# Bill9125/T2MS

Measured on AMD Instinct MI355X. Metric: generated series/sec (B=256, L=96, 1000-step DDPM), higher is better.
Workload: dtype f32; 1 GPU; configs[1]: DiT denoiser, 1000-step ddpm with CFG (2 forwards/step), B=256/GPU, L=96, cfg_scale=9.0, LA-VAE decode; Philox noise on device; hipGraph=on; sampler lanes=2 (part-batch chains on own streams, include/t2s.h t2s_sampler_set_lanes); global_batch=256, diffusion_steps=1000, parallelism=batch-shard x1, sampler_lanes=2

## Files before the change

### include/t2s.h

```cpp
#ifndef T2S_H
#define T2S_H

#include <stdint.h>

#ifdef __cplusplus
extern "C" {
#endif

#define T2S_OK 0
#define T2S_E_INVALID (-1)
#define T2S_E_HIP (-2)
#define T2S_E_STATE (-3)

#define T2S_D_MODEL 128
#define T2S_N_TOK 480
#define T2S_N_HEADS 4
#define T2S_HEAD_DIM 32
#define T2S_N_BLOCKS 4
#define T2S_LAT_C 64
#define T2S_LAT_W 30
#define T2S_LAT_ELEMS (T2S_LAT_C * T2S_LAT_W)

const char* t2s_last_error(void);
const char* t2s_version(void);

typedef struct t2s_dit t2s_dit;

typedef struct t2s_dit_block_weights {
    const float* qkv_w;
    const float* qkv_b;
    const float* proj_w;
    const float* proj_b;
    const float* fc1_w;
    const float* fc1_b;
    const float* fc2_w;
    const float* fc2_b;
    const float* ada_w;
    const float* ada_b;
} t2s_dit_block_weights;

typedef struct t2s_dit_weights {
    const float* conv_w;
    const float* conv_b;
    const float* patch_w;
    const float* patch_b;
    const float* pos_embed;
    const float* ln_w;
    const float* ln_b;
    const float* out_w;
    const float* out_b;
    const float* time_freqs;
    t2s_dit_block_weights blk[T2S_N_BLOCKS];
} t2s_dit_weights;

int t2s_dit_create(const t2s_dit_weights* w, int max_seqs, t2s_dit** out);
#define T2S_DIT_N_TENSORS (10 + 10 * T2S_N_BLOCKS)
int t2s_dit_weights_check(const t2s_dit_weights* w, const uint64_t* n_floats, int n_entries);
int t2s_dit_update_weights(t2s_dit* h, const t2s_dit_weights* w, void* stream);
void t2s_dit_destroy(t2s_dit* h);
int t2s_dit_max_seqs(const t2s_dit* h);
#define T2S_MATH_F32 0
#define T2S_MATH_BF16X3 1
#define T2S_MATH_BF16 2
int t2s_dit_set_math(t2s_dit* h, int math);

int t2s_time_embedding(const t2s_dit* h, const float* t, float* out, int B, void* stream);
int t2s_time_embedding_freqs(const float* freqs, const float* t, float* out, int B, void* stream);

int t2s_dit_forward(t2s_dit* h, const float* x, const float* temb, int temb_rows,
                    const float* text, float* out, int B, void* stream);

int t2s_dit_forward_cfg(t2s_dit* h, const float* x, const float* temb, const float* text,
                        float* out_uncond, float* out_cond, int B, void* stream);
int t2s_dit_forward_cfg_rows(t2s_dit* h, const float* x, const float* temb, int temb_rows, const float* text,
                             float* out_uncond, float* out_cond, int B, void* stream);

int t2s_dit_timing_begin(t2s_dit* h);
int t2s_dit_timing_end(t2s_dit* h, double* out6);
int t2s_dit_timing_end_ex(t2s_dit* h, double* out, int n_classes);

int t2s_dit_read_stream(const t2s_dit* h, float* out, int S, void* stream);

int t2s_attn_fwd(const float* q, const float* k, const float* v, float* o, int BH, void* stream);
int t2s_attn_fwd_packed(const float* q, const float* k, const float* vT, float* o, int n_seq,
                        void* stream);

int t2s_attn_fwd_x3(const float* q, const float* k, const float* v, float* o, int BH, void* stream);

int t2s_attn_fwd_bf16p(const float* q, const float* k, const float* v, float* o, int BH, void* stream);

typedef struct t2s_dit_block_grads {
    float *qkv_w, *qkv_b, *proj_w, *proj_b, *fc1_w, *fc1_b, *fc2_w, *fc2_b, *ada_w, *ada_b;
} t2s_dit_block_grads;
typedef struct t2s_dit_grads {
    float *conv_w, *conv_b, *patch_w, *patch_b, *ln_w, *ln_b, *out_w, *out_b;
    t2s_dit_block_grads blk[T2S_N_BLOCKS];
} t2s_dit_grads;

#define T2S_TRAIN_F32 0
#define T2S_TRAIN_BF16 1
int t2s_dit_set_train_dtype(t2s_dit* h, int dtype);
int t2s_dit_train_forward(t2s_dit* h, const t2s_dit_weights* w, const float* x, const float* temb,
                          int temb_rows, const float* text, float* out, int B, void* stream);
int t2s_attn_fwd_bf16(const float* q, const float* k, const float* v, float* o_rows, float* lse,
                      int n_seq, void* stream);
int t2s_dit_train_backward(t2s_dit* h, const float* dout, const t2s_dit_grads* g, int B, void* stream);
int t2s_dit_train_input_grad(t2s_dit* h, float* dinput, int B, void* stream);
int t2s_adamw_step(float* param, const float* grad, float* exp_avg, float* exp_avg_sq, uint64_t n,
                   float lr, float beta1, float beta2, float eps, float weight_decay, int step,
                   void* stream);
typedef struct t2s_adamw_tensor {
    float* param;
    const float* grad;
    float* exp_avg;
    float* exp_avg_sq;
    uint64_t n;
} t2s_adamw_tensor;
int t2s_adamw_step_multi(const t2s_adamw_tensor* table_dev, int n_tensors, uint64_t total_chunks, float lr,
                         float beta1, float beta2, float eps, float weight_decay, int step, void* stream);
int t2s_mse_backward(const float* a, const float* b, const float* grad_out, float* da, float* db,
                     uint64_t n, void* stream);

int t2s_ddpm_step(float* x, const float* eps_u, const float* eps_c, const float* noise,
                  const float* coef, int t_index, float cfg, uint64_t seed, uint32_t stream_id,
                  uint32_t row0, int B, void* stream);
int t2s_ddpm_p_sample(const float* xt, const float* eps_hat, const int32_t* t, const float* noise,
                      const float* coef, float* out, int B, int n_steps, void* stream);
int t2s_ddpm_p_sample_n(const float* xt, const float* eps_hat, const int32_t* t, const float* noise,
                        const float* coef, float* out, int B, int row_elems, int n_steps, void* stream);
int t2s_ddpm_q_sample_n(const float* x0, const float* eps, const int32_t* t, const float* sqrt_ab,
                        const float* sqrt_1mab, float* out, int B, int row_elems, int n_steps, void* stream);
#define T2S_MSE_SCRATCH_FLOATS 1024
int t2s_mse_ws(const float* a, const float* b, float* out, uint64_t n, float* scratch, void* stream);
int t2s_mse(const float* a, const float* b, float* out, uint64_t n, void* stream);
int t2s_rf_step(float* x, const float* v_u, const float* v_c, float cfg, float dt, int B,
                void* stream);
int t2s_ddpm_q_sample(const float* x0, const float* eps, const int32_t* t, const float* sqrt_ab,
                      const float* sqrt_1mab, float* out, int B, int n_steps, void* stream);
int t2s_rf_create_flow(const float* x1, const float* x0, const float* t, float* out, int B,
                       void* stream);
int t2s_philox_normal(float* out, uint64_t seed, uint32_t stream_id, uint32_t row0, int n_rows,
                      int row_elems, void* stream);
int t2s_philox_normal_rows(float* out, const uint64_t* seeds, const uint32_t* key_rows, uint32_t stream_id,
                           int n_rows, int row_elems, void* stream);
int t2s_philox_uniform(float* out, uint64_t seed, uint32_t stream_id, uint32_t row0, int n_rows,
                       int row_elems, void* stream);

typedef struct t2s_vae t2s_vae;

typedef struct t2s_vae_stack_weights {
    const float* conv3_w[4];
    const float* conv1_w[4];
} t2s_vae_stack_weights;

typedef struct t2s_vae_weights {
    int hidden;
    int res_hidden;
    int n_res_layers;
    int emb;
    const float* dec_conv1_w;
    const float* dec_conv1_b;
    t2s_vae_stack_weights dec_stack;
    const float* dec_ct1_w;
    const float* dec_ct1_b;
    const float* dec_ct2_w;
    const float* dec_ct2_b;
    const float* enc_conv1_w;
    const float* enc_conv1_b;
// ... 124 lines not shown
```

### t2ms_amd/_lib.py

```python
from __future__ import annotations

import ctypes as C
import os
from typing import Optional

import torch

_HERE = os.path.dirname(os.path.abspath(__file__))
LIB_PATH = os.environ.get("T2S_LIB", os.path.join(_HERE, "libt2s_hip.so"))

N_BLOCKS = 4
LAT_C, LAT_W, LAT = 64, 30, 1920
D_MODEL, N_TOK = 128, 480
TRAIN_F32, TRAIN_BF16 = 0, 1
MATH_F32, MATH_BF16X3, MATH_BF16 = 0, 1, 2
MATH_CODES = {"f32": MATH_F32, "bf16x3": MATH_BF16X3, "bf16": MATH_BF16}
DIT_N_TENSORS = 10 + 10 * N_BLOCKS
MSE_SCRATCH_FLOATS = 1024

c_float_p = C.c_void_p


class DitBlockWeights(C.Structure):
    _fields_ = [(n, C.c_void_p) for n in
# ... 38 lines not shown

TS2VEC_MAX_BLOCKS = 16


class Ts2vecWeights(C.Structure):
    _fields_ = [("input_dims", C.c_int), ("hidden", C.c_int), ("output_dims", C.c_int), ("depth", C.c_int),
                ("fc_w", C.c_void_p), ("fc_b", C.c_void_p),
                ("conv1_w", C.c_void_p * TS2VEC_MAX_BLOCKS), ("conv1_b", C.c_void_p * TS2VEC_MAX_BLOCKS),
                ("conv2_w", C.c_void_p * TS2VEC_MAX_BLOCKS), ("conv2_b", C.c_void_p * TS2VEC_MAX_BLOCKS),
                ("proj_w", C.c_void_p), ("proj_b", C.c_void_p)]


MLP_LAYERS, MLP_PACKED_FLOATS = 8, 397888
MLP_LAYER_FIELDS = (("value_w", "cross_attn.value.weight"), ("value_b", "cross_attn.value.bias"),
                    ("proj_w", "cross_attn.proj.weight"), ("proj_b", "cross_attn.proj.bias"),
                    ("norm2_w", "norm2.weight"), ("norm2_b", "norm2.bias"),
                    ("mlp0_w", "mlp.0.weight"), ("mlp0_b", "mlp.0.bias"), ("mlp2_w", "mlp.2.weight"), ("mlp2_b", "mlp.2.bias"),
                    ("pos0_w", "mlp2.0.weight"), ("pos0_b", "mlp2.0.bias"), ("pos2_w", "mlp2.2.weight"), ("pos2_b", "mlp2.2.bias"))


class MlpLayerWeights(C.Structure):
    _fields_ = [(f, C.c_void_p) for f, _ in MLP_LAYER_FIELDS]


class MlpWeights(C.Structure):
    _fields_ = [("layer", MlpLayerWeights * MLP_LAYERS)]


MLP_GRAD_PART_FLOATS = 391744


class MlpGrads(C.Structure):
    _fields_ = [("layer", MlpLayerWeights * MLP_LAYERS)]


class SampleConfig(C.Structure):
    _fields_ = [("mode", C.c_int), ("steps", C.c_int), ("cfg_scale", C.c_float), ("batch", C.c_int),
                ("length", C.c_int), ("use_graph", C.c_int), ("seed", C.c_uint64), ("row0", C.c_uint32),
                ("ddpm_coef", C.c_void_p), ("t_values", C.c_void_p)]


MODE_DDPM, MODE_RF = 0, 1

_VP, _I, _F, _U64, _U32 = C.c_void_p, C.c_int, C.c_float, C.c_uint64, C.c_uint32
SYMBOLS = {
    "t2s_last_error": (C.c_char_p, []),
    "t2s_version": (C.c_char_p, []),
    "t2s_dit_create": (_I, [C.POINTER(DitWeights), _I, C.POINTER(_VP)]),
    "t2s_dit_update_weights": (_I, [_VP, C.POINTER(DitWeights), _VP]),
    "t2s_dit_destroy": (None, [_VP]),
    "t2s_dit_max_seqs": (_I, [_VP]),
    "t2s_time_embedding": (_I, [_VP, _VP, _VP, _I, _VP]),
    "t2s_time_embedding_freqs": (_I, [_VP, _VP, _VP, _I, _VP]),
    "t2s_dit_weights_check": (_I, [C.POINTER(DitWeights), C.POINTER(C.c_uint64), _I]),
    "t2s_dit_forward": (_I, [_VP, _VP, _VP, _I, _VP, _VP, _I, _VP]),
    "t2s_dit_forward_cfg": (_I, [_VP, _VP, _VP, _VP, _VP, _VP, _I, _VP]),
    "t2s_dit_forward_cfg_rows": (_I, [_VP, _VP, _VP, _I, _VP, _VP, _VP, _I, _VP]),
    "t2s_dit_read_stream": (_I, [_VP, _VP, _I, _VP]),
    "t2s_dit_timing_begin": (_I, [_VP]),
    "t2s_dit_timing_end": (_I, [_VP, C.POINTER(C.c_double)]),
    "t2s_dit_timing_end_ex": (_I, [_VP, C.POINTER(C.c_double), _I]),
    "t2s_dit_set_train_dtype": (_I, [_VP, _I]),
    "t2s_dit_set_math": (_I, [_VP, _I]),
    "t2s_eval_mse_wape": (_I, [_VP, _VP, _VP, _VP, _I, _I, _VP]),
    "t2s_eval_mrr": (_I, [_VP, _VP, _VP, _VP, _VP, _I, _I, _I, _F, _VP]),
    "t2s_eval_ed": (_I, [_VP, _VP, _VP, _VP, _I, _I, _I, _VP]),
    "t2s_eval_crps": (_I, [_VP, _VP, _VP, _VP, _I, _I, _I, _I, _VP]),
    "t2s_eval_dtw": (_I, [_VP, _VP, _VP, _VP, _I, _I, _I, _VP]),
    "t2s_ts2vec_encode": (_I, [C.POINTER(Ts2vecWeights), _VP, _VP, _VP, _I, _I, _VP]),
    "t2s_mlp_pack": (_I, [C.POINTER(MlpWeights), _VP, _VP]),
    "t2s_mlp_forward": (_I, [_VP, _VP, _VP, _VP, _VP, _VP, _I, _VP]),
    "t2s_mlp_backward": (_I, [C.POINTER(MlpWeights), _VP, _VP, _VP, _VP, _VP, _VP, _VP, C.POINTER(MlpGrads), _VP, _U64, _I, _VP]),
    "t2s_attn_fwd_x3": (_I, [_VP, _VP, _VP, _VP, _I, _VP]),
    "t2s_attn_fwd_bf16p": (_I, [_VP, _VP, _VP, _VP, _I, _VP]),
    "t2s_attn_fwd_bf16": (_I, [_VP, _VP, _VP, _VP, _VP, _I, _VP]),
    "t2s_dit_train_forward": (_I, [_VP, C.POINTER(DitWeights), _VP, _VP, _I, _VP, _VP, _I, _VP]),
    "t2s_dit_train_backward": (_I, [_VP, _VP, C.POINTER(DitGrads), _I, _VP]),
    "t2s_dit_train_input_grad": (_I, [_VP, _VP, _I, _VP]),
    "t2s_adamw_step": (_I, [_VP, _VP, _VP, _VP, _U64, _F, _F, _F, _F, _F, _I, _VP]),
    "t2s_adamw_step_multi": (_I, [_VP, _I, _U64, _F, _F, _F, _F, _F, _I, _VP]),
    "t2s_mse_backward": (_I, [_VP, _VP, _VP, _VP, _VP, _U64, _VP]),
    "t2s_attn_fwd": (_I, [_VP, _VP, _VP, _VP, _I, _VP]),
    "t2s_attn_fwd_packed": (_I, [_VP, _VP, _VP, _VP, _I, _VP]),
    "t2s_ddpm_step": (_I, [_VP, _VP, _VP, _VP, _VP, _I, _F, _U64, _U32, _U32, _I, _VP]),
    "t2s_ddpm_p_sample": (_I, [_VP, _VP, _VP, _VP, _VP, _VP, _I, _I, _VP]),
    "t2s_ddpm_p_sample_n": (_I, [_VP, _VP, _VP, _VP, _VP, _VP, _I, _I, _I, _VP]),
    "t2s_ddpm_q_sample_n": (_I, [_VP, _VP, _VP, _VP, _VP, _VP, _I, _I, _I, _VP]),
    "t2s_vae_decode_w": (_I, [_VP, _VP, _VP, _VP, _I, _I, _I, _VP]),
    "t2s_mse": (_I, [_VP, _VP, _VP, _U64, _VP]),
    "t2s_mse_ws": (_I, [_VP, _VP, _VP, _U64, _VP, _VP]),
    "t2s_rf_step": (_I, [_VP, _VP, _VP, _F, _F, _I, _VP]),
    "t2s_ddpm_q_sample": (_I, [_VP, _VP, _VP, _VP, _VP, _VP, _I, _I, _VP]),
    "t2s_rf_create_flow": (_I, [_VP, _VP, _VP, _VP, _I, _VP]),
    "t2s_philox_normal": (_I, [_VP, _U64, _U32, _U32, _I, _I, _VP]),
    "t2s_philox_uniform": (_I, [_VP, _U64, _U32, _U32, _I, _I, _VP]),
    "t2s_vae_create": (_I, [C.POINTER(VaeWeights), C.POINTER(_VP)]),
    "t2s_vae_destroy": (None, [_VP]),
    "t2s_vae_update_weights": (_I, [_VP, C.POINTER(VaeWeights), _VP]),
    "t2s_vae_encode_backward": (_I, [_VP, _VP, _VP, _VP, C.POINTER(VaeEncGrads), _I, _I, _VP]),
    "t2s_vae_decode": (_I, [_VP, _VP, _VP, _VP, _I, _I, _VP]),
    "t2s_vae_encode": (_I, [_VP, _VP, _VP, _VP, _I, _I, _VP]),
    "t2s_sampler_create": (_I, [_VP, _VP, C.POINTER(SampleConfig), C.POINTER(_VP)]),
    "t2s_sampler_destroy": (None, [_VP]),
    "t2s_sampler_run": (_I, [_VP, _VP, _VP, _VP, _VP, _VP, _VP]),
    "t2s_sampler_set_lanes": (_I, [_VP, _I]),
    "t2s_sampler_set_loop_graph": (_I, [_VP, _I]),
    "t2s_sampler_set_row0": (_I, [_VP, _U32]),
    "t2s_sampler_set_rows": (_I, [_VP, _VP, _VP, _VP, _I]),
    "t2s_philox_normal_rows": (_I, [_VP, _VP, _VP, _U32, _I, _I, _VP]),
    "t2s_sampler_graph_lanes": (_I, [_VP]),
    "t2s_sampler_lane_pool": (_I, []),
}

_lib: Optional[C.CDLL] = None


class T2SError(RuntimeError):
    pass


def lib() -> C.CDLL:
    global _lib
    if _lib is None:
        if not os.path.exists(LIB_PATH):
            raise T2SError(
                f"{LIB_PATH} is missing: build it with `python -c 'import __graft_entry__ as g; g.build()'` "
                f"or `make -C t2ms_amd/csrc` (hipcc --offload-arch=gfx950).  There is no CPU fallback.")
        handle = C.CDLL(LIB_PATH)
        for name, (res, args) in SYMBOLS.items():
            fn = getattr(handle, name)
            fn.restype, fn.argtypes = res, args
        _lib = handle
    return _lib


def check(rc: int, what: str = "") -> None:
    if rc != 0:
        msg = lib().t2s_last_error().decode("utf-8", "replace")
        raise T2SError(f"{what or 't2s call'} failed (rc={rc}): {msg}")


def dev_ptr(t: Optional[torch.Tensor], name: str = "tensor", dtype=torch.float32) -> Optional[int]:
    if t is None:
        return None
    if not t.is_cuda:
        raise T2SError(f"{name} must live on a GPU (got device {t.device}); the HIP path has no CPU fallback")
    if t.dtype != dtype:
        raise T2SError(f"{name} must be {dtype} (got {t.dtype})")
    if not t.is_contiguous():
        raise T2SError(f"{name} must be contiguous")
    return t.data_ptr()


def as_f32(t: torch.Tensor) -> torch.Tensor:
    if t.dtype != torch.float32:
        t = t.float()
    return t.contiguous()


_DEVICE_LOCKS = {}


def device_lock(device) -> "threading.RLock":
    import threading
    return _DEVICE_LOCKS.setdefault(str(torch.device(device)), threading.RLock())

# ... 9 lines not shown
```

### t2ms_amd/csrc/t2s_attn.hip

```cpp
#include <stdlib.h>

#include "t2s_common.h"

namespace t2s {

struct SoftmaxState {
    float m_run;
    float l_lane;
};

__device__ __forceinline__ float pair_max(float v) {
    const auto r = __builtin_amdgcn_permlane32_swap(__float_as_uint(v), __float_as_uint(v), false, false);
    return fmaxf(__uint_as_float(r[0]), __uint_as_float(r[1]));
}
__device__ __forceinline__ float pair_sum(float v) {
    const auto r = __builtin_amdgcn_permlane32_swap(__float_as_uint(v), __float_as_uint(v), false, false);
    return __uint_as_float(r[0]) + __uint_as_float(r[1]);
}

__device__ __forceinline__ void softmax_block(f32x16& st, f32x16& ot, SoftmaxState& s) {
    float mloc = st[0];
#pragma unroll
    for (int r = 1; r < 16; ++r) mloc = fmaxf(mloc, st[r]);
    mloc = pair_max(mloc);
    const float m_new = fmaxf(s.m_run, mloc);
    const float alpha = __builtin_amdgcn_exp2f(s.m_run - m_new);
    s.m_run = m_new;
    float psum = 0.f;
#pragma unroll
    for (int r = 0; r < 16; ++r) {
        st[r] = __builtin_amdgcn_exp2f(st[r] - m_new);
        psum += st[r];
    }
    s.l_lane = s.l_lane * alpha + psum;
#pragma unroll
    for (int r = 0; r < 16; ++r) ot[r] *= alpha;
}

constexpr float QSCALE = 0.17677669529663687f * 1.4426950408889634f;

constexpr int ATT_SLOTS = 4;
constexpr int ATT_SLOT_F4 = 512;
constexpr int ATT_LDS_BYTES = ATT_SLOTS * ATT_SLOT_F4 * 16;
constexpr int NKB = NTOK / 32;

constexpr float SM_BIG = 1.152921504606847e18f;


struct TileState {
    f32x16 negm;
    float m_ref;
    float l_lane;
};

__device__ __forceinline__ float exp_sum(f32x16& st) {
#pragma unroll
    for (int r = 0; r < 16; ++r) st[r] = __builtin_amdgcn_exp2f(st[r]);
    return ((st[0] + st[1]) + (st[2] + st[3])) + ((st[4] + st[5]) + (st[6] + st[7])) +
           (((st[8] + st[9]) + (st[10] + st[11])) + ((st[12] + st[13]) + (st[14] + st[15])));
}

__device__ __forceinline__ float rereference(const f32x4 (&kf)[4], const f32x4 (&q)[4], f32x16& st,
                                             f32x16& ot, TileState& t) {
#pragma unroll
    for (int r = 0; r < 16; ++r) st[r] = 0.f;
#pragma unroll
    for (int g = 0; g < 4; ++g)
#pragma unroll
        for (int e = 0; e < 4; ++e) st = mfma32(kf[g][e], q[g][e], st);
    float mloc = st[0];
#pragma unroll
    for (int r = 1; r < 16; ++r) mloc = fmaxf(mloc, st[r]);
    mloc = pair_max(mloc);
    const float m_new = fmaxf(t.m_ref, mloc);
    const float alpha = __builtin_amdgcn_exp2f(t.m_ref - m_new);
    t.m_ref = m_new;
    t.l_lane *= alpha;
#pragma unroll
    for (int r = 0; r < 16; ++r) {
        ot[r] *= alpha;
        t.negm[r] = -m_new;
        st[r] -= m_new;
    }
    return exp_sum(st);
}
// ... 218 lines not shown
                        sta = mfma32(kf[g][e], qa[g][e], sta);
                        if (NT == 2) stb = mfma32(kf[g][e], qb[g][e], stb);
                    }
                psa = exp_sum(sta);
                if (NT == 2) psb = exp_sum(stb);
                const bool stale = !(psa < SM_BIG) || !(psb < SM_BIG);
                redo = __builtin_amdgcn_ballot_w64(stale) != 0;
            }
            if (redo) {
                psa = rereference(kf, qa, sta, oa, ta);
                if (NT == 2) psb = rereference(kf, qb, stb, ob, tb);
            }
            ta.l_lane += psa;
            tb.l_lane += psb;
#pragma unroll
            for (int g = 0; g < 4; ++g)
#pragma unroll
                for (int e = 0; e < 4; ++e) oa = mfma32(vf[g][e], sta[4 * g + e], oa);
            if (jb == NKB - 4 && bh + stride < BH) {
                const f32x4* qg = qall + (size_t)(bh + stride) * NKB * 256;
#pragma unroll
                for (int g = 0; g < 4; ++g) {
                    qna[g] = qg[(t0 * 4 + g) * 64 + lane];
                    if (NT == 2) qnb[g] = qg[((t0 + 1) * 4 + g) * 64 + lane];
                }
            }
            ATT_PERSIST_WAIT();
            __builtin_amdgcn_s_barrier();
            issue_block(bh, jb + 4, gb + 4);
            {
                const f32x4* nslot = ring + ((gb + 1) & (ATT_SLOTS - 1)) * ATT_SLOT_F4 + lane;
#pragma unroll
                for (int g = 0; g < 4; ++g) kf[g] = nslot[g * 64];
            }
            if (NT == 2) {
#pragma unroll
                for (int g = 0; g < 4; ++g)
#pragma unroll
                    for (int e = 0; e < 4; ++e) ob = mfma32(vf[g][e], stb[4 * g + e], ob);
            }
        }
        const int seq = bh / NH, head = bh % NH;
        {
            const float inv = 1.0f / pair_sum(ta.l_lane);
#pragma unroll
            for (int g = 0; g < 4; ++g) {
                const f32x4 w = {oa[4 * g] * inv, oa[4 * g + 1] * inv, oa[4 * g + 2] * inv, oa[4 * g + 3] * inv};
                og[(((size_t)seq * NKB + t0) * 16 + head * 4 + g) * 64 + lane] = w;
            }
        }
        if (NT == 2) {
            const float inv = 1.0f / pair_sum(tb.l_lane);
#pragma unroll
            for (int g = 0; g < 4; ++g) {
                const f32x4 w = {ob[4 * g] * inv, ob[4 * g + 1] * inv, ob[4 * g + 2] * inv, ob[4 * g + 3] * inv};
                og[(((size_t)seq * NKB + t0 + 1) * 16 + head * 4 + g) * 64 + lane] = w;
            }
        }
#pragma unroll
        for (int g = 0; g < 4; ++g) {
            qa[g] = qna[g] * QSCALE;
            if (NT == 2) qb[g] = qnb[g] * QSCALE;
        }
    }
    asm volatile("s_waitcnt vmcnt(0)" ::: "memory");
}

__global__ __launch_bounds__(PERSIST_THREADS, 2) void attn_fwd_persistent_kernel(
    const float* __restrict__ q, const float* __restrict__ k, const float* __restrict__ vT,
    float* __restrict__ o, int BH) {
    extern __shared__ __attribute__((aligned(16))) f32x4 ring[];
    const int lane = threadIdx.x & 63;
    const int wave = __builtin_amdgcn_readfirstlane(threadIdx.x >> 6);
    const f32x4* qg = reinterpret_cast<const f32x4*>(q);
    const f32x4* kg = reinterpret_cast<const f32x4*>(k);
    const f32x4* vg = reinterpret_cast<const f32x4*>(vT);
    f32x4* og = reinterpret_cast<f32x4*>(o);
    if (wave < 7)
        attn_persistent_body<2>(ring, qg, kg, vg, og, BH, lane, wave);
    else
        attn_persistent_body<1>(ring, qg, kg, vg, og, BH, lane, wave);
}

int launch_attn_packed(const float* q, const float* k, const float* vT, float* o, int BH, hipStream_t st) {
    static int n_cu = 0;
    if (n_cu == 0) {
        int dev = 0;
        hipDeviceProp_t prop;
        if (hipGetDevice(&dev) == hipSuccess && hipGetDeviceProperties(&prop, dev) == hipSuccess)
            n_cu = prop.multiProcessorCount;
        else
            n_cu = 256;
    }
    static const int persist_min = getenv("T2S_ATTN_PERSIST_MIN") ? atoi(getenv("T2S_ATTN_PERSIST_MIN")) : 0;
    if (BH >= (persist_min > 0 ? persist_min : 3 * n_cu)) {
        attn_fwd_persistent_kernel<<<BH < n_cu ? BH : n_cu, PERSIST_THREADS, ATT_LDS_BYTES, st>>>(q, k, vT, o, BH);
    } else {
        static const int parts_env = getenv("T2S_ATTN_PARTS") ? atoi(getenv("T2S_ATTN_PARTS")) : 0;
        const int parts = parts_env == 2 || parts_env == 4 ? parts_env : (((BH + 7) / 8) * 16 < n_cu ? 4 : 2);
        if (parts == 4)
            attn_fwd_packed_kernel<4><<<((BH + 7) / 8) * 32, 256, ATT_LDS_BYTES, st>>>(q, k, vT, o, BH);
        else
            attn_fwd_packed_kernel<2><<<((BH + 7) / 8) * 16, 256, ATT_LDS_BYTES, st>>>(q, k, vT, o, BH);
    }
    T2S_LAUNCH_CHECK();
    return T2S_OK;
}

constexpr int KSTR = 36;
constexpr int PLAIN_LDS_BYTES = (NTOK * KSTR + NTOK * DH) * 4;

__global__ __launch_bounds__(512) void attn_fwd_plain_kernel(const float* __restrict__ q,
                                                             const float* __restrict__ k,
                                                             const float* __restrict__ v,
                                                             float* __restrict__ o) {
    extern __shared__ __attribute__((aligned(16))) float smem[];
    float* Ks = smem;
    float* Vs = smem + NTOK * KSTR;
    const int bh = blockIdx.x;
    const int tid = threadIdx.x;
    const int lane = tid & 63, wave = tid >> 6, half = lane >> 5, i = lane & 31;
    const float* kg = k + (size_t)bh * NTOK * DH;
    const float* vg = v + (size_t)bh * NTOK * DH;
    const float* qg = q + (size_t)bh * NTOK * DH;
    for (int idx = tid; idx < NTOK * DH / 4; idx += 512) {
        const f32x4 kv = reinterpret_cast<const f32x4*>(kg)[idx];
        const f32x4 vv = reinterpret_cast<const f32x4*>(vg)[idx];
        const int row = idx >> 3, col = (idx & 7) * 4;
        *reinterpret_cast<f32x4*>(Ks + row * KSTR + col) = kv;
        *reinterpret_cast<f32x4*>(Vs + row * DH + col) = vv;
    }
    __syncthreads();
    for (int qt = wave; qt < NKB; qt += 8) {
        f32x4 qf[4];
#pragma unroll
        for (int g = 0; g < 4; ++g)
            qf[g] = *reinterpret_cast<const f32x4*>(qg + (size_t)(qt * 32 + i) * DH + 8 * g + 4 * half) * QSCALE;
        f32x16 ot;
#pragma unroll
        for (int r = 0; r < 16; ++r) ot[r] = 0.f;
        SoftmaxState s{-INFINITY, 0.f};
        for (int jb = 0; jb < NKB; ++jb) {
            f32x16 st;
#pragma unroll
            for (int r = 0; r < 16; ++r) st[r] = 0.f;
            const float* krow = Ks + (jb * 32 + i) * KSTR + 4 * half;
#pragma unroll
            for (int g = 0; g < 4; ++g) {
                const f32x4 kf = *reinterpret_cast<const f32x4*>(krow + 8 * g);
#pragma unroll
                for (int e = 0; e < 4; ++e) st = mfma32(kf[e], qf[g][e], st);
            }
            softmax_block(st, ot, s);
            const float* vrow = Vs + (jb * 32 + 4 * half) * DH + i;
#pragma unroll
            for (int r = 0; r < 16; ++r) {
                const int klo = (r & 3) + 8 * (r >> 2);
                ot = mfma32(vrow[klo * DH], st[r], ot);
            }
        }
        const float inv = 1.0f / pair_sum(s.l_lane);
#pragma unroll
        for (int g = 0; g < 4; ++g) {
            const f32x4 w = {ot[4 * g] * inv, ot[4 * g + 1] * inv, ot[4 * g + 2] * inv, ot[4 * g + 3] * inv};
            *reinterpret_cast<f32x4*>(o + ((size_t)bh * NTOK + qt * 32 + i) * DH + 8 * g + 4 * half) = w;
        }
    }
}

int attn_init() {
    static bool attr_set = false;
    if (!attr_set) {
        T2S_HIP_CHECK(hipFuncSetAttribute(reinterpret_cast<const void*>(attn_fwd_plain_kernel),
                                          hipFuncAttributeMaxDynamicSharedMemorySize, PLAIN_LDS_BYTES));
        attr_set = true;
    }
    return T2S_OK;
}

}

extern "C" int t2s_attn_fwd(const float* q, const float* k, const float* v, float* o, int BH,
                            void* stream) {
    T2S_REQUIRE(q && k && v && o, "t2s_attn_fwd: NULL pointer");
    T2S_REQUIRE(BH > 0, "t2s_attn_fwd: BH=%d must be > 0", BH);
    if (int rc = t2s::attn_init()) return rc;
    t2s::attn_fwd_plain_kernel<<<BH, 512, t2s::PLAIN_LDS_BYTES, (hipStream_t)stream>>>(q, k, v, o);
    T2S_LAUNCH_CHECK();
    return T2S_OK;
}


extern "C" int t2s_attn_fwd_packed(const float* q, const float* k, const float* vT, float* o, int n_seq,
                                   void* stream) {
    T2S_REQUIRE(q && k && vT && o, "t2s_attn_fwd_packed: NULL pointer");
    T2S_REQUIRE(n_seq > 0, "t2s_attn_fwd_packed: n_seq=%d must be > 0", n_seq);
    return t2s::launch_attn_packed(q, k, vT, o, n_seq * t2s::NH, (hipStream_t)stream);
}
```

Before: 64.40 series/s.

## Add fill-scheduled persistent attention kernel that packs tiles across heads

Adds a persistent attention kernel in which each CTA processes its heads in epochs. Groups of 16 heads are spread so that 15 query tiles per head fill the 8 waves, and wave 7 takes a donor tile from the group's last head. The goal is to remove idle waves, since each head has 15 tiles but a CTA has 16 tile slots. The fill kernel becomes the default path for large BH, with an env switch back to the old kernel and host-side plan/job query functions for checking. The cost is much more complex scheduling code, extra global loads for donor K/V, and more register pressure.

```diff
diff --git a/include/t2s.h b/include/t2s.h
--- a/include/t2s.h
+++ b/include/t2s.h
@@ -84,6 +84,8 @@
 int t2s_attn_fwd(const float* q, const float* k, const float* v, float* o, int BH, void* stream);
 int t2s_attn_fwd_packed(const float* q, const float* k, const float* vT, float* o, int n_seq,
                         void* stream);
+int t2s_attn_fill_plan(int n_heads, int head, int tile, int* out);
+int t2s_attn_fill_job(int n_heads, int epoch, int wave, int slot, int* out);
 
 int t2s_attn_fwd_x3(const float* q, const float* k, const float* v, float* o, int BH, void* stream);
 
diff --git a/t2ms_amd/_lib.py b/t2ms_amd/_lib.py
--- a/t2ms_amd/_lib.py
+++ b/t2ms_amd/_lib.py
@@ -144,6 +144,8 @@
     "t2s_mse_backward": (_I, [_VP, _VP, _VP, _VP, _VP, _U64, _VP]),
     "t2s_attn_fwd": (_I, [_VP, _VP, _VP, _VP, _I, _VP]),
     "t2s_attn_fwd_packed": (_I, [_VP, _VP, _VP, _VP, _I, _VP]),
+    "t2s_attn_fill_plan": (_I, [_I, _I, _I, C.POINTER(_I)]),
+    "t2s_attn_fill_job": (_I, [_I, _I, _I, _I, C.POINTER(_I)]),
     "t2s_ddpm_step": (_I, [_VP, _VP, _VP, _VP, _VP, _I, _F, _U64, _U32, _U32, _I, _VP]),
     "t2s_ddpm_p_sample": (_I, [_VP, _VP, _VP, _VP, _VP, _VP, _I, _I, _VP]),
     "t2s_ddpm_p_sample_n": (_I, [_VP, _VP, _VP, _VP, _VP, _VP, _I, _I, _I, _VP]),
diff --git a/t2ms_amd/csrc/t2s_attn.hip b/t2ms_amd/csrc/t2s_attn.hip
--- a/t2ms_amd/csrc/t2s_attn.hip
+++ b/t2ms_amd/csrc/t2s_attn.hip
@@ -1,6 +1,7 @@
 #include <stdlib.h>
 
 #include "t2s_common.h"
+#include "t2s_attn_fill.h"
 
 namespace t2s {
 
@@ -385,6 +386,422 @@
         attn_persistent_body<1>(ring, qg, kg, vg, og, BH, lane, wave);
 }
 
+template <bool W7>
+__device__ __forceinline__ void attn_fill_body(f32x4* ring, const f32x4* qall, const f32x4* kall, const f32x4* vall,
+                                               f32x4* og, int BH, int lane, int wave) {
+    constexpr size_t HEAD_F4 = (size_t)NKB * 256;
+    const int stride = gridDim.x;
+    const int first = blockIdx.x;
+    const int n = (BH - first + stride - 1) / stride;
+    const int n_epochs = attn_fill_epochs(n);
+
+    int rh, rh_next = -1;
+    int gb = 0;
+    auto issue_block = [&](int jb, int gslot) {
+        int bh = rh;
+        if (jb >= NKB) {
+            if (rh_next >= 0) { bh = rh_next; jb -= NKB; }
+            else jb = NKB - 1;
+        }
+        const size_t off = bh * HEAD_F4 + jb * 256 + (wave & 3) * 64 + lane;
+        glds16_asm((wave < 4 ? kall : vall) + off, ring + (gslot & (ATT_SLOTS - 1)) * ATT_SLOT_F4 + wave * 64);
+    };
+
+    AttnFillEpoch ep = attn_fill_epoch(n, 0);
+    int start, cnt;
+    attn_fill_wave_tiles(ep.ring_tiles, wave, &start, &cnt);
+    rh = first + ep.ring_head * stride;
+    bool mixed = W7 && ep.donor_head >= 0;
+    int tA = cnt >= 1 ? ep.ring_t0 + start : 0;
+    int dh = mixed ? first + ep.donor_head * stride : rh;
+    int tB = mixed ? ep.donor_tile : (cnt == 2 ? tA + 1 : 0);
+    issue_block(0, 0);
+    issue_block(1, 1);
+    issue_block(2, 2);
+
+    f32x4 qa[4], qb[4], kd[4], kf[4];
+#pragma unroll
+    for (int g = 0; g < 4; ++g) {
+        kd[g] = f32x4{0.f, 0.f, 0.f, 0.f};
+        qa[g] = qall[rh * HEAD_F4 + (tA * 4 + g) * 64 + lane] * QSCALE;
+        qb[g] = qall[dh * HEAD_F4 + (tB * 4 + g) * 64 + lane] * QSCALE;
+        if constexpr (W7) kd[g] = kall[dh * HEAD_F4 + g * 64 + lane];
+    }
+    if constexpr (W7)
+        asm volatile("s_waitcnt vmcnt(0)" ::: "memory");
+    else
+        asm volatile("s_waitcnt vmcnt(2)" ::: "memory");
+    __builtin_amdgcn_s_barrier();
+    issue_block(3, 3);
+#pragma unroll
+    for (int g = 0; g < 4; ++g) kf[g] = ring[g * 64 + lane];
+
+#pragma unroll 1
+    for (int epoch = 0; epoch < n_epochs; ++epoch) {
+        const bool more = epoch + 1 < n_epochs;
+        const AttnFillEpoch nx = attn_fill_epoch(n, more ? epoch + 1 : epoch);
+        int nstart, ncnt;
+        attn_fill_wave_tiles(nx.ring_tiles, wave, &nstart, &ncnt);
+        if (!more) ncnt = 0;
+        rh_next = more ? first + nx.ring_head * stride : -1;
+        const int rhn = more ? rh_next : rh;
+        const bool nmixed = W7 && more && nx.donor_head >= 0;
+        const int ntA = ncnt >= 1 ? nx.ring_t0 + nstart : 0;
+        const int ndh = nmixed ? first + nx.donor_head * stride : rhn;
+        const int ntB = nmixed ? nx.donor_tile : (ncnt == 2 ? ntA + 1 : 0);
+        const f32x4* qan = qall + rhn * HEAD_F4 + ntA * 256;
+        const f32x4* qbn = qall + ndh * HEAD_F4 + ntB * 256;
+
+        auto run = [&](auto nt_c, auto mixed_c) __attribute__((always_inline)) {
+            constexpr int NT = decltype(nt_c)::value;
+            constexpr bool MIXED = decltype(mixed_c)::value;
+            constexpr bool HAS_B = NT == 2 || MIXED;
+            f32x16 oa, ob;
+            TileState ta, tb;
+#pragma unroll
+            for (int r = 0; r < 16; ++r) {
+                oa[r] = ob[r] = 0.f;
+                ta.negm[r] = tb.negm[r] = INFINITY;
+            }
+            ta.m_ref = tb.m_ref = -INFINITY;
+            ta.l_lane = tb.l_lane = 0.f;
+            const f32x4* kdg = kall + dh * HEAD_F4;
+            const f32x4* vdg = vall + dh * HEAD_F4;
+#define ATT_KB(g) (MIXED ? kd[g] : kf[g])
+#define ATT_VB(g) (MIXED ? vd[g] : vf[g])
+
+            auto step = [&](int jb, auto last_c) __attribute__((always_inline)) {
+                constexpr bool LAST = decltype(last_c)::value;
+                const f32x4* slot = ring + (gb & (ATT_SLOTS - 1)) * ATT_SLOT_F4 + lane;
+                f32x4 vf[4], vd[4];
+                if constexpr (NT >= 1) {
+#pragma unroll
+                    for (int g = 0; g < 4; ++g) vf[g] = slot[256 + g * 64];
+                }
+                if constexpr (MIXED) {
+#pragma unroll
+                    for (int g = 0; g < 4; ++g) vd[g] = vdg[jb * 256 + g * 64 + lane];
+                }
+                f32x16 sta = ta.negm, stb = tb.negm;
+                if constexpr (NT >= 1) {
+                    float psa = 0.f, psb = 0.f;
+                    bool redo = jb == 0;
+                    if (!redo) {
+                        sta = mfma32_from(kf[0][0], qa[0][0], ta.negm);
+                        if (HAS_B) stb = mfma32_from(ATT_KB(0)[0], qb[0][0], tb.negm);
+#pragma unroll
+                        for (int g = 0; g < 4; ++g)
+#pragma unroll
+                            for (int e = (g == 0 ? 1 : 0); e < 4; ++e) {
+                                sta = mfma32(kf[g][e], qa[g][e], sta);
+                                if (HAS_B) stb = mfma32(ATT_KB(g)[e], qb[g][e], stb);
+                            }
+                        psa = exp_sum(sta);
+                        if (HAS_B) psb = exp_sum(stb);
+                        const bool stale = !(psa < SM_BIG) || !(psb < SM_BIG);
+                        redo = __builtin_amdgcn_ballot_w64(stale) != 0;
+                    }
+                    if (redo) {
+                        psa = rereference(kf, qa, sta, oa, ta);
+                        if constexpr (MIXED) psb = rereference(kd, qb, stb, ob, tb);
+                        else if constexpr (NT == 2) psb = rereference(kf, qb, stb, ob, tb);
+                    }
+                    ta.l_lane += psa;
+                    tb.l_lane += psb;
+                }
+                {
+                    if constexpr (W7 && (MIXED || LAST)) {
+                        const f32x4* kp = LAST ? kall + ndh * HEAD_F4 : kdg + (jb + 1) * 256;
+#pragma unroll
+                        for (int g = 0; g < 4; ++g) kd[g] = kp[g * 64 + lane];
+                    }
+                    if constexpr (LAST) {
+#pragma unroll
+                        for (int g = 0; g < 4; ++g) {
+                            qa[g] = qan[g * 64 + lane];
+                            qb[g] = qbn[g * 64 + lane];
+                        }
+                    }
+                }
+                if constexpr (NT >= 1) {
+#pragma unroll
+                    for (int g = 0; g < 4; ++g)
+#pragma unroll
+                        for (int e = 0; e < 4; ++e) oa = mfma32(vf[g][e], sta[4 * g + e], oa);
+                }
+                if constexpr (MIXED) {
+                    if (jb < 2) asm volatile("s_waitcnt vmcnt(14)" ::: "memory");
+                    else asm volatile("s_waitcnt vmcnt(26)" ::: "memory");
+                } else if constexpr (NT == 0) {
+                    asm volatile("s_waitcnt vmcnt(2) lgkmcnt(0)" ::: "memory");
+                } else {
+                    asm volatile("s_waitcnt vmcnt(2)" ::: "memory");
+                }
+                __builtin_amdgcn_s_barrier();
+                issue_block(jb + 4, gb + 4);
+                {
+                    const f32x4* nslot = ring + ((gb + 1) & (ATT_SLOTS - 1)) * ATT_SLOT_F4 + lane;
+#pragma unroll
+                    for (int g = 0; g < 4; ++g) kf[g] = nslot[g * 64];
+                }
+                if constexpr (HAS_B) {
+#pragma unroll
+                    for (int g = 0; g < 4; ++g)
+#pragma unroll
+                        for (int e = 0; e < 4; ++e) ob = mfma32(ATT_VB(g)[e], stb[4 * g + e], ob);
+                }
+                ++gb;
+            };
+#pragma unroll 1
+            for (int jb = 0; jb < NKB - 1; ++jb) step(jb, std::false_type{});
+            step(NKB - 1, std::true_type{});
+#undef ATT_KB
+#undef ATT_VB
+            if constexpr (NT >= 1) {
+                const int seq = rh / NH, head = rh % NH;
+                const float inv = 1.0f / pair_sum(ta.l_lane);
+#pragma unroll
+                for (int g = 0; g < 4; ++g) {
+                    const f32x4 w = {oa[4 * g] * inv, oa[4 * g + 1] * inv, oa[4 * g + 2] * inv, oa[4 * g + 3] * inv};
+                    og[(((size_t)seq * NKB + tA) * 16 + head * 4 + g) * 64 + lane] = w;
+                }
+            }
+            if constexpr (HAS_B) {
+                const int seq = dh / NH, head = dh % NH;
+                const float inv = 1.0f / pair_sum(tb.l_lane);
+#pragma unroll
+                for (int g = 0; g < 4; ++g) {
+                    const f32x4 w = {ob[4 * g] * inv, ob[4 * g + 1] * inv, ob[4 * g + 2] * inv, ob[4 * g + 3] * inv};
+                    og[(((size_t)seq * NKB + tB) * 16 + head * 4 + g) * 64 + lane] = w;
+                }
+            }
+        };
+        using std::integral_constant;
+        if constexpr (W7) {
+            if (mixed) run(integral_constant<int, 1>{}, integral_constant<bool, true>{});
+            else if (cnt == 1) run(integral_constant<int, 1>{}, integral_constant<bool, false>{});
+            else run(integral_constant<int, 0>{}, integral_constant<bool, false>{});
+        } else {
+            if (cnt == 2) run(integral_constant<int, 2>{}, integral_constant<bool, false>{});
+            else if (cnt == 1) run(integral_constant<int, 1>{}, integral_constant<bool, false>{});
+            else run(integral_constant<int, 0>{}, integral_constant<bool, false>{});
+        }
+#pragma unroll
+        for (int g = 0; g < 4; ++g) {
+            qa[g] *= QSCALE;
+            qb[g] *= QSCALE;
+            asm volatile("" ::"v"(qa[g]), "v"(qb[g]));
+            if constexpr (W7) asm volatile("" ::"v"(kd[g]));
+        }
+        rh = rhn; cnt = ncnt; mixed = nmixed; tA = ntA; dh = ndh; tB = ntB;
+    }
+    asm volatile("s_waitcnt vmcnt(0)" ::: "memory");
+}
+
+__global__ __launch_bounds__(PERSIST_THREADS, 2) void attn_fwd_persistent_fill_kernel(
+    const float* __restrict__ q, const float* __restrict__ k, const float* __restrict__ vT,
+    float* __restrict__ o, int BH) {
+    extern __shared__ __attribute__((aligned(16))) f32x4 ring[];
+    const int lane = threadIdx.x & 63;
+    const int wave = __builtin_amdgcn_readfirstlane(threadIdx.x >> 6);
+    const f32x4* qg = reinterpret_cast<const f32x4*>(q);
+    const f32x4* kg = reinterpret_cast<const f32x4*>(k);
+    const f32x4* vg = reinterpret_cast<const f32x4*>(vT);
+    f32x4* og = reinterpret_cast<f32x4*>(o);
+    if (wave < 7)
+        attn_fill_body<false>(ring, qg, kg, vg, og, BH, lane, wave);
+    else
+        attn_fill_body<true>(ring, qg, kg, vg, og, BH, lane, wave);
+}
+
+#ifdef T2S_ATTN_FILL_BOUND
+template <bool MIXED>
+__device__ __forceinline__ void attn_fillbound_body(f32x4* ring, const f32x4* qall, const f32x4* kall,
+                                                    const f32x4* vall, f32x4* og, int BH, int lane, int wave) {
+    const int stride = gridDim.x;
+    const int t0 = wave * 2;
+    const int t1 = MIXED ? t0 : t0 + 1;
+    auto donor = [&](int h) { return MIXED && h + stride < BH ? h + stride : h; };
+    auto issue_block = [&](int bh, int jb, int gslot) {
+        if (jb >= NKB) { jb -= NKB; bh += stride; }
+        if (bh >= BH) { bh -= stride; jb = NKB - 1; }
+        const size_t off = (size_t)bh * NKB * 256 + jb * 4 * 64 + (wave & 3) * 64 + lane;
+        glds16_asm((wave < 4 ? kall : vall) + off, ring + (gslot & (ATT_SLOTS - 1)) * ATT_SLOT_F4 + wave * 64);
+    };
+    int bh = blockIdx.x;
+    int gb = 0;
+    issue_block(bh, 0, 0);
+    issue_block(bh, 1, 1);
+    issue_block(bh, 2, 2);
+
+    f32x4 qa[4], qb[4], qna[4], qnb[4], kd[4], vd[4];
+    {
+        const f32x4* qg = qall + (size_t)bh * NKB * 256;
+        const f32x4* qd = qall + (size_t)donor(bh) * NKB * 256;
+        const f32x4* kg = kall + (size_t)donor(bh) * NKB * 256;
+#pragma unroll
+        for (int g = 0; g < 4; ++g) {
+            qa[g] = qg[(t0 * 4 + g) * 64 + lane] * QSCALE;
+            qb[g] = qd[(t1 * 4 + g) * 64 + lane] * QSCALE;
+            qna[g] = qa[g];
+            qnb[g] = qb[g];
+            if (MIXED) kd[g] = kg[g * 64 + lane];
+        }
+    }
+    if constexpr (MIXED)
+        asm volatile("s_waitcnt vmcnt(0)" ::: "memory");
+    else
+        asm volatile("s_waitcnt vmcnt(2)" ::: "memory");
+    __builtin_amdgcn_s_barrier();
+    issue_block(bh, 3, 3);
+    f32x4 kf[4];
+#pragma unroll
+    for (int g = 0; g < 4; ++g) kf[g] = ring[g * 64 + lane];
+
+#pragma unroll 1
+    for (; bh < BH; bh += stride) {
+        f32x16 oa, ob;
+        TileState ta, tb;
+#pragma unroll
+        for (int r = 0; r < 16; ++r) {
+            oa[r] = ob[r] = 0.f;
+            ta.negm[r] = tb.negm[r] = INFINITY;
+        }
+        ta.m_ref = tb.m_ref = -INFINITY;
+        ta.l_lane = tb.l_lane = 0.f;
+        const int dh = donor(bh);
+
+#pragma unroll 1
+        for (int jb = 0; jb < NKB; ++jb, ++gb) {
+            const f32x4* slot = ring + (gb & (ATT_SLOTS - 1)) * ATT_SLOT_F4 + lane;
+            f32x4 vf[4];
+#pragma unroll
+            for (int g = 0; g < 4; ++g) vf[g] = slot[256 + g * 64];
+            if constexpr (MIXED) {
+                const f32x4* vg = vall + (size_t)dh * NKB * 256 + jb * 256 + lane;
+#pragma unroll
+                for (int g = 0; g < 4; ++g) vd[g] = vg[g * 64];
+            }
+#define ATT_KB(g) (MIXED ? kd[g] : kf[g])
+#define ATT_VB(g) (MIXED ? vd[g] : vf[g])
+            f32x16 sta = ta.negm, stb = tb.negm;
+            float psa = 0.f, psb = 0.f;
+            bool redo = jb == 0;
+            if (!redo) {
+                sta = mfma32_from(kf[0][0], qa[0][0], ta.negm);
+                stb = mfma32_from(ATT_KB(0)[0], qb[0][0], tb.negm);
+#pragma unroll
+                for (int g = 0; g < 4; ++g)
+#pragma unroll
+                    for (int e = (g == 0 ? 1 : 0); e < 4; ++e) {
+                        sta = mfma32(kf[g][e], qa[g][e], sta);
+                        stb = mfma32(ATT_KB(g)[e], qb[g][e], stb);
+                    }
+                psa = exp_sum(sta);
+                psb = exp_sum(stb);
+                const bool stale = !(psa < SM_BIG) || !(psb < SM_BIG);
+                redo = __builtin_amdgcn_ballot_w64(stale) != 0;
+            }
+            if (redo) {
+                psa = rereference(kf, qa, sta, oa, ta);
+                if constexpr (MIXED) psb = rereference(kd, qb, stb, ob, tb);
+                else psb = rereference(kf, qb, stb, ob, tb);
+            }
+            ta.l_lane += psa;
+            tb.l_lane += psb;
+            if constexpr (MIXED) {
+                const bool last = jb == NKB - 1;
+                const int nh = last && bh + stride < BH ? bh + stride : bh;
+                const f32x4* kg = kall + (size_t)donor(nh) * NKB * 256 + (last ? 0 : jb + 1) * 256 + lane;
+#pragma unroll
+                for (int g = 0; g < 4; ++g) kd[g] = kg[g * 64];
+                if (last) {
+                    const f32x4* qg = qall + (size_t)nh * NKB * 256;
+                    const f32x4* qd = qall + (size_t)donor(nh) * NKB * 256;
+#pragma unroll
+                    for (int g = 0; g < 4; ++g) {
+                        qa[g] = qg[(t0 * 4 + g) * 64 + lane];
+                        qb[g] = qd[(t1 * 4 + g) * 64 + lane];
+                    }
+                }
+            }
+#pragma unroll
+            for (int g = 0; g < 4; ++g)
+#pragma unroll
+                for (int e = 0; e < 4; ++e) oa = mfma32(vf[g][e], sta[4 * g + e], oa);
+            if constexpr (MIXED)
+                asm volatile("s_waitcnt vmcnt(26)" ::: "memory");
+            else
+                asm volatile("s_waitcnt vmcnt(2)" ::: "memory");
+            __builtin_amdgcn_s_barrier();
+            issue_block(bh, jb + 4, gb + 4);
+            if (!MIXED && jb == NKB - 4 && bh + stride < BH) {
+                const f32x4* qg = qall + (size_t)(bh + stride) * NKB * 256;
+#pragma unroll
+                for (int g = 0; g < 4; ++g) {
+                    qna[g] = qg[(t0 * 4 + g) * 64 + lane];
+                    qnb[g] = qg[(t1 * 4 + g) * 64 + lane];
+                }
+            }
+            {
+                const f32x4* nslot = ring + ((gb + 1) & (ATT_SLOTS - 1)) * ATT_SLOT_F4 + lane;
+#pragma unroll
+                for (int g = 0; g < 4; ++g) kf[g] = nslot[g * 64];
+            }
+#pragma unroll
+            for (int g = 0; g < 4; ++g)
+#pragma unroll
+                for (int e = 0; e < 4; ++e) ob = mfma32(ATT_VB(g)[e], stb[4 * g + e], ob);
+#undef ATT_KB
+#undef ATT_VB
+        }
+        {
+            const int seq = bh / NH, head = bh % NH;
+            const float inv = 1.0f / pair_sum(ta.l_lane);
+#pragma unroll
+            for (int g = 0; g < 4; ++g) {
+                const f32x4 w = {oa[4 * g] * inv, oa[4 * g + 1] * inv, oa[4 * g + 2] * inv, oa[4 * g + 3] * inv};
+                og[(((size_t)seq * NKB + t0) * 16 + head * 4 + g) * 64 + lane] = w;
+            }
+        }
+        {
+            const int seq = dh / NH, head = dh % NH;
+            const float inv = 1.0f / pair_sum(tb.l_lane);
+#pragma unroll
+            for (int g = 0; g < 4; ++g) {
+                const f32x4 w = {ob[4 * g] * inv, ob[4 * g + 1] * inv, ob[4 * g + 2] * inv, ob[4 * g + 3] * inv};
+                og[(((size_t)seq * NKB + t1) * 16 + head * 4 + g) * 64 + lane] = w;
+            }
+        }
+#pragma unroll
+        for (int g = 0; g < 4; ++g) {
+            qa[g] = (MIXED ? qa[g] : qna[g]) * QSCALE;
+            qb[g] = (MIXED ? qb[g] : qnb[g]) * QSCALE;
+        }
+    }
+    asm volatile("s_waitcnt vmcnt(0)" ::: "memory");
+}
+
+__global__ __launch_bounds__(PERSIST_THREADS, 2) void attn_fwd_persistent_fillbound_kernel(
+    const float* __restrict__ q, const float* __restrict__ k, const float* __restrict__ vT,
+    float* __restrict__ o, int BH) {
+    extern __shared__ __attribute__((aligned(16))) f32x4 ring[];
+    const int lane = threadIdx.x & 63;
+    const int wave = __builtin_amdgcn_readfirstlane(threadIdx.x >> 6);
+    const f32x4* qg = reinterpret_cast<const f32x4*>(q);
+    const f32x4* kg = reinterpret_cast<const f32x4*>(k);
+    const f32x4* vg = reinterpret_cast<const f32x4*>(vT);
+    f32x4* og = reinterpret_cast<f32x4*>(o);
+    if (wave < 7)
+        attn_fillbound_body<false>(ring, qg, kg, vg, og, BH, lane, wave);
+    else
+        attn_fillbound_body<true>(ring, qg, kg, vg, og, BH, lane, wave);
+}
+#define T2S_ATTN_FILL_KERNEL attn_fwd_persistent_fillbound_kernel
+#else
+#define T2S_ATTN_FILL_KERNEL attn_fwd_persistent_fill_kernel
+#endif
+
 int launch_attn_packed(const float* q, const float* k, const float* vT, float* o, int BH, hipStream_t st) {
     static int n_cu = 0;
     if (n_cu == 0) {
@@ -397,7 +814,11 @@
     }
     static const int persist_min = getenv("T2S_ATTN_PERSIST_MIN") ? atoi(getenv("T2S_ATTN_PERSIST_MIN")) : 0;
     if (BH >= (persist_min > 0 ? persist_min : 3 * n_cu)) {
-        attn_fwd_persistent_kernel<<<BH < n_cu ? BH : n_cu, PERSIST_THREADS, ATT_LDS_BYTES, st>>>(q, k, vT, o, BH);
+        static const int fill = getenv("T2S_ATTN_FILL") ? atoi(getenv("T2S_ATTN_FILL")) : 1;
+        if (fill)
+            T2S_ATTN_FILL_KERNEL<<<BH < n_cu ? BH : n_cu, PERSIST_THREADS, ATT_LDS_BYTES, st>>>(q, k, vT, o, BH);
+        else
+            attn_fwd_persistent_kernel<<<BH < n_cu ? BH : n_cu, PERSIST_THREADS, ATT_LDS_BYTES, st>>>(q, k, vT, o, BH);
     } else {
         static const int parts_env = getenv("T2S_ATTN_PARTS") ? atoi(getenv("T2S_ATTN_PARTS")) : 0;
         const int parts = parts_env == 2 || parts_env == 4 ? parts_env : (((BH + 7) / 8) * 16 < n_cu ? 4 : 2);
@@ -500,3 +921,21 @@
     T2S_REQUIRE(n_seq > 0, "t2s_attn_fwd_packed: n_seq=%d must be > 0", n_seq);
     return t2s::launch_attn_packed(q, k, vT, o, n_seq * t2s::NH, (hipStream_t)stream);
 }
+
+extern "C" int t2s_attn_fill_plan(int n_heads, int head, int tile, int* out) {
+    T2S_REQUIRE(out, "t2s_attn_fill_plan: NULL pointer");
+    T2S_REQUIRE(n_heads > 0 && head >= 0 && head < n_heads && tile >= 0 && tile < t2s::ATT_FILL_TILES,
+                "t2s_attn_fill_plan: (n_heads=%d, head=%d, tile=%d) out of range", n_heads, head, tile);
+    t2s::attn_fill_plan(n_heads, head, tile, out, out + 1, out + 2);
+    return T2S_OK;
+}
+
+extern "C" int t2s_attn_fill_job(int n_heads, int epoch, int wave, int slot, int* out) {
+    T2S_REQUIRE(out, "t2s_attn_fill_job: NULL pointer");
+    T2S_REQUIRE(n_heads > 0 && epoch >= 0 && wave >= 0 && wave < 8 && slot >= 0 && slot < 2,
+                "t2s_attn_fill_job: (n_heads=%d, epoch=%d, wave=%d, slot=%d) out of range", n_heads, epoch, wave, slot);
+    const int n_epochs = t2s::attn_fill_epochs(n_heads);
+    if (epoch >= n_epochs) return n_epochs;
+    t2s::attn_fill_job(n_heads, epoch, wave, slot, out, out + 1);
+    return n_epochs;
+}
diff --git a/t2ms_amd/csrc/t2s_attn_fill.h b/t2ms_amd/csrc/t2s_attn_fill.h
--- /dev/null
+++ b/t2ms_amd/csrc/t2s_attn_fill.h
@@ -0,0 +1,66 @@
+#pragma once
+
+namespace t2s {
+
+constexpr int ATT_FILL_TILES = 15;
+constexpr int ATT_FILL_GROUP = 16;
+
+struct AttnFillEpoch {
+    int ring_head;
+    int ring_t0;
+    int ring_tiles;
+    int donor_head;
+    int donor_tile;
+};
+
+__host__ __device__ inline int attn_fill_epochs(int n) { return n - n / ATT_FILL_GROUP; }
+
+__host__ __device__ inline AttnFillEpoch attn_fill_epoch(int n, int epoch) {
+    const int full = n / ATT_FILL_GROUP;
+    const int grp = epoch < full * (ATT_FILL_GROUP - 1) ? epoch / (ATT_FILL_GROUP - 1) : full;
+    const int e = epoch - grp * (ATT_FILL_GROUP - 1);
+    const int g = grp < full ? ATT_FILL_GROUP : n - full * ATT_FILL_GROUP;
+    const int h0 = grp * ATT_FILL_GROUP;
+    if (e < g - 1) return {h0 + e, 0, ATT_FILL_TILES, h0 + g - 1, e};
+    return {h0 + g - 1, g - 1, ATT_FILL_GROUP - g, -1, 0};
+}
+
+__host__ __device__ inline void attn_fill_wave_tiles(int tiles, int wave, int* start, int* count) {
+    const int second = tiles > 8 ? tiles - 8 : 0;
+    *count = (tiles > wave) + (second > wave);
+    *start = (wave < tiles ? wave : tiles) + (wave < second ? wave : second);
+}
+
+__host__ __device__ inline void attn_fill_plan(int n, int head, int tile, int* epoch, int* wave, int* slot) {
+    const int full = n / ATT_FILL_GROUP;
+    const int grp = head / ATT_FILL_GROUP;
+    const int g = grp < full ? ATT_FILL_GROUP : n - full * ATT_FILL_GROUP;
+    const int j = head - grp * ATT_FILL_GROUP;
+    const int e0 = grp * (ATT_FILL_GROUP - 1);
+    int idx = tile, tiles = ATT_FILL_TILES;
+    if (j < g - 1) {
+        *epoch = e0 + j;
+    } else if (tile < g - 1) {
+        *epoch = e0 + tile; *wave = 7; *slot = 1;
+        return;
+    } else {
+        *epoch = e0 + g - 1; idx = tile - (g - 1); tiles = ATT_FILL_GROUP - g;
+    }
+    for (int w = 0; w < 8; ++w) {
+        int start, count;
+        attn_fill_wave_tiles(tiles, w, &start, &count);
+        if (idx >= start && idx < start + count) { *wave = w; *slot = idx - start; return; }
+    }
+    *wave = *slot = -1;
+}
+
+__host__ __device__ inline void attn_fill_job(int n, int epoch, int wave, int slot, int* head, int* tile) {
+    const AttnFillEpoch ep = attn_fill_epoch(n, epoch);
+    int start, count;
+    attn_fill_wave_tiles(ep.ring_tiles, wave, &start, &count);
+    *head = -1; *tile = -1;
+    if (slot < count) { *head = ep.ring_head; *tile = ep.ring_t0 + start + slot; }
+    else if (wave == 7 && slot == 1 && ep.donor_head >= 0) { *head = ep.donor_head; *tile = ep.donor_tile; }
+}
+
+}
```

Measured after the change: 64.95 series/s (median of 6 runs). Within noise of the previous version (+0.9%).
